# adaly/gridnext

Measured on AMD Instinct MI355X. Metric: spots/sec training throughput (multimodal f+g), higher is better.
Workload: dtype f32; 1 GPU; C4: multimodal f(DenseNet-121 @128px + count-MLP 2000 genes) + hex g on 78x64 Visium grids, 1 array (4992 spots) per GPU per step, f frozen/eval (tutorial mode), g trained with Adam, masked CE; spots_per_array=4992, parallelism=dp1

## Files before the change

### gridnext_amd/_lib.py

```python
import ctypes
import os

import torch

_HERE = os.path.dirname(os.path.abspath(__file__))
LIB_PATH = os.environ.get('GNX_LIB') or os.path.join(_HERE, 'libgridnext_hip.so')

_P, _I, _L, _F, _D = ctypes.c_void_p, ctypes.c_int, ctypes.c_long, ctypes.c_float, ctypes.c_double

SIGNATURES = {
    'gnx_hexconv_fwd': (_I, [_P, _P, _P, _P, _P, _I, _I, _I, _I, _I, _I, _P]),
    'gnx_hexconv_bwd_data': (_I, [_P, _P, _P, _P, _I, _I, _I, _I, _I, _I, _P]),
    'gnx_hexconv_bwd_weight_workspace': (_L, [_I, _I, _I, _I, _I]),
    'gnx_hexconv_bwd_weight': (_I, [_P, _P, _P, _P, _P, _P, _I, _I, _I, _I, _I, _I, _I, _P]),
    'gnx_hexconv_bwd_weight_batch': (_I, [_P, _I, _P]),
    'gnx_hexconv_k_fwd': (_I, [_P, _P, _P, _P, _I, _I, _I, _I, _I, _I, _I, _P]),
    'gnx_hexconv_k_bwd_data': (_I, [_P, _P, _P, _I, _I, _I, _I, _I, _I, _I, _P]),
    'gnx_hexconv_k_bwd_weight_workspace': (_L, [_I, _I, _I, _I, _I, _I]),
    'gnx_hexconv_k_bwd_weight': (_I, [_P, _P, _P, _P, _P, _I, _I, _I, _I, _I, _I, _I, _I, _P]),
    'gnx_bn_workspace': (_L, [_L, _I]),
    'gnx_bn_train_stats': (_I, [_P, _L, _L, _I, _P, _P, _P, _P, _P, _F, _F, _P, _P, _P, _P, _P, _P]),
    'gnx_bn_train_stats_sync': (_I, [_P, _L, _L, _I, _P, _P, _P, _P, _P, _F, _F, _P, _P, _P, _P, _P, _P, _P]),
    'gnx_bn_train_stats_apply': (_I, [_P, _L, _L, _I, _P, _P, _P, _P, _P, _F, _F, _P, _P, _P, _P, _P, _L, _I, _P, _P]),
    'gnx_bn_sync_words': (_L, [_I]),
# ... 78 lines not shown
    'gnx_conv_stem_bnrelu_maxpool_f16mul_cb': (_I, [_P, _I, _P, _P, _L, _L, _I, _I, _I, _I, _I, _I, _I, _I, _P, _P, _P, _P]),
    'gnx_conv1x1_bnrelu_h16_cb': (_I, [_P, _L, _P, _P, _L, _L, _I, _I, _P, _P, _P, _P, _P]),
    'gnx_bnrelu_avgpool2_h16_cb': (_I, [_P, _L, _P, _L, _L, _I, _I, _P, _P, _P]),
    'gnx_transition_f16_pack': (_I, [_P, _P, _I, _I, _P]),
    'gnx_transition_f16': (_I, [_P, _L, _L, _I, _I, _I, _P, _P, _P, _P, _L, _P]),
    'gnx_transition_f16_tape': (_I, [_P, _L, _L, _I, _I, _I, _P, _P, _P, _P, _L, _P, _L, _P]),
    'gnx_bnrelu_avgpool_h16_cb': (_I, [_P, _L, _P, _L, _L, _I, _I, _P, _P, _P]),
    'gnx_conv3x3_bnrelu': (_I, [_P, _L, _P, _P, _L, _L, _I, _I, _I, _P, _P, _P]),
    'gnx_winograd_conv3x3_weights': (_I, [_P, _P, _I, _I, _P]),
    'gnx_conv3x3_winograd': (_I, [_P, _L, _P, _P, _L, _L, _I, _I, _I, _P]),
    'gnx_conv_stem': (_I, [_P, _P, _P, _L, _L, _I, _I, _I, _I, _I, _I, _I, _I, _P]),
    'gnx_conv_stem_bnrelu_maxpool': (_I, [_P, _P, _P, _L, _L, _I, _I, _I, _I, _I, _I, _I, _I, _P, _P, _P]),
    'gnx_conv_stem_bnrelu_maxpool_argmax': (_I, [_P, _P, _P, _L, _P, _L, _I, _I, _I, _I, _I, _I, _I, _I, _P, _P, _P]),
    'gnx_bnrelu_maxpool': (_I, [_P, _L, _P, _L, _L, _I, _I, _I, _P, _P, _P]),
    'gnx_bnrelu_avgpool': (_I, [_P, _L, _P, _L, _L, _I, _I, _P, _P, _P]),
    'gnx_wgrad_workspace': (_L, [_L, _I, _I, _I]),
    'gnx_wgrad_bnrelu': (_I, [_P, _L, _P, _L, _P, _P, _P, _P, _L, _I, _I, _I, _I, _I, _I, _P]),
    'gnx_wgrad_bnrelu_batch': (_I, [_P, _I, _I, _P]),
    'gnx_transpose_weight': (_I, [_P, _P, _I, _I, _P]),
    'gnx_relayout_weights_batch': (_I, [_P, _I, _I, _P]),
    'gnx_repack_conv3x3_bwd': (_I, [_P, _P, _I, _I, _P]),
    'gnx_rows_broadcast': (_I, [_P, _L, _P, _L, _L, _I, _I, _F, _P]),
    'gnx_avgpool2_bwd': (_I, [_P, _L, _P, _L, _L, _I, _I, _P]),
    'gnx_maxpool_bwd': (_I, [_P, _L, _P, _L, _P, _L, _P, _L, _L, _I, _I, _I, _P, _P, _P]),
    'gnx_bnrelu_maxpool_argmax': (_I, [_P, _L, _P, _L, _P, _L, _I, _I, _I, _P, _P, _P]),
    'gnx_maxpool_bwd_argmax': (_I, [_P, _P, _L, _P, _L, _L, _I, _I, _I, _P]),
    'gnx_maxpool_bwd_argmax_bnrelu': (_I, [_P, _P, _L, _P, _L, _P, _P, _L, _L, _I, _I, _I, _P]),
    'gnx_conv0_wgrad_workspace': (_L, [_L, _I, _I, _I, _I, _I, _I, _I]),
    'gnx_conv0_wgrad': (_I, [_P, _P, _L, _P, _P, _L, _I, _I, _I, _I, _I, _I, _I, _I, _P]),
    'gnx_softmax_rows': (_I, [_P, _L, _L, _I, _P, _L, _P, _P]),
# ... 62 lines not shown
```

### gridnext_amd/csrc/stem_pool.hip

```cpp
#include <type_traits>
#include "fwd_common.h"

namespace {

__device__ __forceinline__ float u8_unit(float u) {
    constexpr float R255 = 1.0f / 255.0f;
    const float q = u * R255;
    const float e = fmaf(-255.0f, q, u);
    return fmaf(e, R255, q);
}
__device__ __forceinline__ float u8_pixel(float u, bool norm, float mean, float sd, float rsd) {
    float v = u8_unit(u);
    if (norm) {
        const float t = v - mean;
        const float q = t * rsd;
        const float e = fmaf(-sd, q, t);
        v = fmaf(e, rsd, q);
    }
    return v;
}
__device__ __forceinline__ float4 u8x4_pixels(uint32_t wv, bool norm, float mean, float sd, float rsd) {
    return make_float4(u8_pixel((float)(wv & 0xffu), norm, mean, sd, rsd),
                       u8_pixel((float)((wv >> 8) & 0xffu), norm, mean, sd, rsd),
                       u8_pixel((float)((wv >> 16) & 0xffu), norm, mean, sd, rsd),
// ... 178 lines not shown
                if (i < O) o[i] = acc0[r];
                if (32 + i < O) o[32 + i] = acc1[r];
            }
        }
    }
}

constexpr int SP_LDT = 40;
constexpr int SP_LDTH = 72;
template <int WO, bool H16 = false, bool U8 = false, bool IDX = false>
__global__ __launch_bounds__(256) void conv_stem_pool_kernel(const void* __restrict__ xv, const float* __restrict__ w,
                                                             float* __restrict__ out, long ldo, int H, int Wd, int O,
                                                             const float* __restrict__ scale,
                                                             const float* __restrict__ shift, long imgs,
                                                             const float* __restrict__ nrm,
                                                             unsigned char* __restrict__ amax = nullptr) {
    const float* __restrict__ x = reinterpret_cast<const float*>(xv);
    const uint8_t* __restrict__ x8 = reinterpret_cast<const uint8_t*>(xv);
    constexpr int CIN = 3, KH = 7, KW = 7, STRIDE = 2, PAD = 3;
    constexpr int RT = 128 / WO;
    constexpr int PH = STRIDE * (RT - 1) + KH, PW = ((WO - 1) * STRIDE + 8 + 1 + 1) & ~1;
    constexpr int F4R = WO * STRIDE / 4;
    constexpr int NPC = CIN * PH * F4R, NPRE = (NPC + 255) / 256;
    constexpr int NIT = (WO / 2) * 8 / 256;
    constexpr int KT = CIN * KH * 8, LDB = KT + 4;
    extern __shared__ __attribute__((aligned(16))) float lds[];
    auto store4 = [](float* o, long off, const float4& v) {
        if constexpr (H16) {
            typedef _Float16 half4 __attribute__((ext_vector_type(4)));
            const half4 hv = {(_Float16)v.x, (_Float16)v.y, (_Float16)v.z, (_Float16)v.w};
            *reinterpret_cast<half4*>(reinterpret_cast<_Float16*>(o) + off) = hv;
// ... 51 lines not shown
            if (j < NPC) {
                float* d = Ps + (j / F4R) * PW + PAD + 4 * (j % F4R);
                if constexpr (U8) {
                    const int c = (j / F4R) / PH;
                    const bool norm = nrm != nullptr;
                    const float4 v = in8[q] ? u8x4_pixels(pre8[q], norm, norm ? nrm[c] : 0.f, norm ? nrm[3 + c] : 1.f,
                                                          norm ? nrm[6 + c] : 1.f)
                                            : make_float4(0.f, 0.f, 0.f, 0.f);
                    d[0] = v.x; d[1] = v.y; d[2] = v.z; d[3] = v.w;
                } else {
                    d[0] = pre[q].x; d[1] = pre[q].y; d[2] = pre[q].z; d[3] = pre[q].w;
                }
            }
        }
    };
    __syncthreads();
    fetch_patch(blockIdx.x, 0);

    for (long img = blockIdx.x; img < imgs; img += gridDim.x) {
        float4 carry[2][NIT], carry2[2][NIT];
        unsigned cidx[2][NIT], cidx2[2][NIT];
        const float c0v = IDX ? -1.f : 0.f;
#pragma unroll
        for (int q = 0; q < NIT; ++q) {
            carry[0][q] = carry[1][q] = carry2[0][q] = carry2[1][q] = make_float4(c0v, c0v, c0v, c0v);
            cidx[0][q] = cidx[1][q] = cidx2[0][q] = cidx2[1][q] = 0u;
        }
        for (int tt = 0; tt < ntt; ++tt) {
            __syncthreads();
            stash_patch();
            {
                long nimg = img;
                int nt2 = tt + 1;
                if (nt2 == ntt) { nt2 = 0; nimg += gridDim.x; }
                if (nimg >= imgs) nimg = blockIdx.x;
                fetch_patch(nimg, nt2);
            }
            asm volatile("" ::: "memory");
            __syncthreads();
            f32x16 acc0, acc1;
#pragma unroll
            for (int r = 0; r < 16; ++r) { acc0[r] = 0.f; acc1[r] = 0.f; }
            auto load_a = [&](int step) {
                const float* ap = pa + ((step / KH) * PH + (step % KH)) * PW;
                const float2 lo = *reinterpret_cast<const float2*>(ap);
                const float2 hi = *reinterpret_cast<const float2*>(ap + 2);
                return make_float4(lo.x, lo.y, hi.x, hi.y);
            };
            constexpr int NSTEP = CIN * KH;
            float4 a = load_a(0), b0 = ld4(pb), b1 = ld4(pb + 32 * LDB);
#pragma unroll
// ... 356 lines not shown
                    if (a2 > m.z) { m.z = a2; am = (am & 0xff00ffffu) | (li << 16); }
                    if (a3 > m.w) { m.w = a3; am = (am & 0x00ffffffu) | (li << 24); }
                } else {
                    m.x = fmaxf(m.x, a0); m.y = fmaxf(m.y, a1); m.z = fmaxf(m.z, a2); m.w = fmaxf(m.w, a3);
                }
            }
        }
        *reinterpret_cast<float4*>(out + row * ldo + c) = m;
        if (IDX) *reinterpret_cast<unsigned*>(amax + row * (4L * C4) + c) = am;
    }
}

template <bool IN16 = false>
__global__ __launch_bounds__(256) void bnrelu_avgpool_kernel(const float* __restrict__ in, long ldi, float* __restrict__ out,
                                                             long ldo, int C, int S2, const float* __restrict__ scale,
                                                             const float* __restrict__ shift, long ibs = 32) {
    __shared__ float red[4][64];
    const int cl = threadIdx.x & 63, rl = threadIdx.x >> 6;
    const int c = blockIdx.y * 64 + cl;
    const long img = blockIdx.x;
    float acc = 0.f;
    if (c < C) {
        const float sc = scale[c], sh = shift[c];
        for (int r = rl; r < S2; r += 4) {
            const long off = (img * S2 + r) * ldi + (c >> 5) * ibs + (c & 31);
            const float v = IN16 ? (float)reinterpret_cast<const _Float16*>(in)[off] : in[off];
            acc += fmaxf(fmaf(v, sc, sh), 0.f);
        }
    }
    red[rl][cl] = acc;
    __syncthreads();
    if (rl == 0 && c < C)
        out[img * ldo + c] = ((red[0][cl] + red[1][cl]) + (red[2][cl] + red[3][cl])) / (float)S2;
}

}

GNX_EXPORT int gnx_conv_stem(const float* x, const float* w, float* out, long ldc, long imgs, int Cin, int H, int W,
                             int O, int KH, int KW, int stride, int pad, hipStream_t stream) {
    if (!x || !w || !out || imgs < 0 || Cin <= 0 || O <= 0 || KH <= 0 || KH > 7 || KW <= 0 || KW > 8 || stride <= 0 ||
        ldc < O)
        return GNX_ERR_BAD_ARG;
    const int Ho = (H + 2 * pad - KH) / stride + 1, Wo = (W + 2 * pad - KW) / stride + 1;
    if (Ho <= 0 || Wo <= 0) return GNX_ERR_BAD_ARG;
    const long M = imgs * Ho * Wo;
    if (M == 0) return GNX_OK;
    if (O <= 64 && Cin == 3 && ((stride == 2 && KH == 7 && KW == 7) || (stride == 1 && KH == 3 && KW == 3))) {
        const int tiles_x = gnx_cdiv(Wo, 16), tiles_y = gnx_cdiv(Ho, 8);
// ... 6 lines not shown
                                                                      tiles_x, tiles_y, ntiles);
        else
            conv_stem_patch_kernel<1, 3, 3><<<grid2, 256, lds2, stream>>>(x, w, out, ldc, Cin, H, W, Ho, Wo, O, KW, pad,
                                                                      tiles_x, tiles_y, ntiles);
        return gnx_launch_status();
    }
    const size_t lds_bytes = (size_t)(ST_BM + ST_BN) * (KH * 8 + 4) * sizeof(float);
    dim3 grid(gnx_cdiv(M, ST_BM), gnx_cdiv(O, ST_BN));
    conv_stem_kernel<<<grid, 256, lds_bytes, stream>>>(x, w, out, ldc, M, Cin, H, W, Ho, Wo, O, KH, KW, stride, pad);
    return gnx_launch_status();
}

template <bool H16, bool U8 = false>
static int stem_pool_launch(const void* x, const float* w, float* out, long ldo, long imgs, int Cin, int H, int W, int O,
                            int KH, int KW, int stride, int pad, const float* scale, const float* shift, hipStream_t stream,
                            const float* nrm = nullptr, unsigned char* amax = nullptr) {
    if (!x || !w || !out || !scale || !shift || imgs < 0 || Cin <= 0 || O <= 0 || H <= 0 || W <= 0 || ldo < O)
        return GNX_ERR_BAD_ARG;
    if (amax && (H16 || U8 || (reinterpret_cast<uintptr_t>(amax) & 3) != 0)) return GNX_ERR_UNSUPPORTED;
    if (Cin != 3 || KH != 7 || KW != 7 || stride != 2 || pad != 3 || O > 64 || O % 4 != 0 || ldo % 4 != 0 ||
        (reinterpret_cast<uintptr_t>(out) & (H16 ? 7 : 15)) != 0)
        return GNX_ERR_UNSUPPORTED;
    const int Ho = (H + 6 - 7) / 2 + 1, Wo = (W + 6 - 7) / 2 + 1;
    if ((Wo != 64 && Wo != 128) || W != 2 * Wo || Ho % 2 != 0 || Ho <= 0 ||
        (reinterpret_cast<uintptr_t>(x) & (U8 ? 3 : 15)) != 0)
        return GNX_ERR_UNSUPPORTED;
    if (imgs == 0) return GNX_OK;
    const int RT = 128 / Wo, PH = 2 * (RT - 1) + 7, PW = ((Wo - 1) * 2 + 8 + 2) & ~1;
    const size_t lds_bytes = ((size_t)64 * (3 * 7 * 8 + 4) + (size_t)3 * PH * PW + (size_t)128 * SP_LDT) * sizeof(float);
    const int per_cu = lds_bytes <= 80 * 1024 ? 2 : 1;
    const int grid = (int)(imgs < 256 * per_cu ? imgs : 256 * per_cu);
    if (Wo == 64) {
        static bool conf = false;
// ... 5 lines not shown
        }
        if constexpr (!H16 && !U8) {
            if (amax) {
                static bool confi = false;
                if (!confi) {
                    if (hipFuncSetAttribute(reinterpret_cast<const void*>(conv_stem_pool_kernel<64, false, false, true>),
                                            hipFuncAttributeMaxDynamicSharedMemorySize, (int)lds_bytes) != hipSuccess)
                        return GNX_ERR_LAUNCH;
                    confi = true;
                }
                conv_stem_pool_kernel<64, false, false, true><<<grid, 256, lds_bytes, stream>>>(x, w, out, ldo, H, W, O, scale,
                                                                                                shift, imgs, nrm, amax);
                return gnx_launch_status();
            }
        }
        conv_stem_pool_kernel<64, H16, U8><<<grid, 256, lds_bytes, stream>>>(x, w, out, ldo, H, W, O, scale, shift, imgs, nrm);
    } else {
        static bool conf = false;
        if (!conf) {
            if (hipFuncSetAttribute(reinterpret_cast<const void*>(conv_stem_pool_kernel<128, H16, U8>),
                                    hipFuncAttributeMaxDynamicSharedMemorySize, (int)lds_bytes) != hipSuccess)
                return GNX_ERR_LAUNCH;
            conf = true;
        }
        if constexpr (!H16 && !U8) {
            if (amax) {
                static bool confi = false;
                if (!confi) {
                    if (hipFuncSetAttribute(reinterpret_cast<const void*>(conv_stem_pool_kernel<128, false, false, true>),
                                            hipFuncAttributeMaxDynamicSharedMemorySize, (int)lds_bytes) != hipSuccess)
                        return GNX_ERR_LAUNCH;
                    confi = true;
                }
                conv_stem_pool_kernel<128, false, false, true><<<grid, 256, lds_bytes, stream>>>(x, w, out, ldo, H, W, O, scale,
                                                                                                 shift, imgs, nrm, amax);
                return gnx_launch_status();
            }
        }
        conv_stem_pool_kernel<128, H16, U8><<<grid, 256, lds_bytes, stream>>>(x, w, out, ldo, H, W, O, scale, shift, imgs, nrm);
    }
    return gnx_launch_status();
}
GNX_EXPORT int gnx_conv_stem_bnrelu_maxpool(const float* x, const float* w, float* out, long ldo, long imgs, int Cin,
                                            int H, int W, int O, int KH, int KW, int stride, int pad, const float* scale,
                                            const float* shift, hipStream_t stream) {
    return stem_pool_launch<false>(x, w, out, ldo, imgs, Cin, H, W, O, KH, KW, stride, pad, scale, shift, stream);
}
GNX_EXPORT int gnx_conv_stem_bnrelu_maxpool_argmax(const float* x, const float* w, float* out, long ldo,
                                                   unsigned char* argmax, long imgs, int Cin, int H, int W, int O, int KH,
                                                   int KW, int stride, int pad, const float* scale, const float* shift,
                                                   hipStream_t stream) {
    if (!argmax) return GNX_ERR_BAD_ARG;
    return stem_pool_launch<false>(x, w, out, ldo, imgs, Cin, H, W, O, KH, KW, stride, pad, scale, shift, stream, nullptr,
                                   argmax);
}
GNX_EXPORT int gnx_conv_stem_bnrelu_maxpool_h16(const float* x, const float* w, void* out16, long ldo, long imgs, int Cin,
                                                int H, int W, int O, int KH, int KW, int stride, int pad,
                                                const float* scale, const float* shift, hipStream_t stream) {
    return stem_pool_launch<true>(x, w, reinterpret_cast<float*>(out16), ldo, imgs, Cin, H, W, O, KH, KW, stride, pad, scale,
                                  shift, stream);
}
// ... 44 lines not shown
    if (norm) return GNX_ERR_BAD_ARG;
    return stem_pool_f16_launch<false>(x, w, out16, 32, imgs, Cin, H, W, O, KH, KW, stride, pad, scale, shift, nullptr, stream,
                                       rows_total * 32);
}

GNX_EXPORT int gnx_conv_stem_bnrelu_maxpool_u8(const uint8_t* x8, const float* w, void* out, long ldo, long imgs, int Cin,
                                               int H, int W, int O, int KH, int KW, int stride, int pad, const float* scale,
                                               const float* shift, const float* norm, int out_f16, hipStream_t stream) {
    if (out_f16)
        return stem_pool_launch<true, true>(x8, w, reinterpret_cast<float*>(out), ldo, imgs, Cin, H, W, O, KH, KW, stride, pad,
                                            scale, shift, stream, norm);
    return stem_pool_launch<false, true>(x8, w, reinterpret_cast<float*>(out), ldo, imgs, Cin, H, W, O, KH, KW, stride, pad,
                                         scale, shift, stream, norm);
}

GNX_EXPORT int gnx_u8_to_f32(const uint8_t* x8, float* out, long imgs, int C, int H, int W, const float* norm,
                             hipStream_t stream) {
    if (!x8 || !out || imgs < 0 || C <= 0 || H <= 0 || W <= 0 || (norm && C != 3)) return GNX_ERR_BAD_ARG;
    const long hw = (long)H * W;
    if (hw % 4 != 0 || (reinterpret_cast<uintptr_t>(x8) & 3) != 0 || !al16(out)) return GNX_ERR_UNSUPPORTED;
    const long n4 = imgs * C * hw / 4;
    if (n4 == 0) return GNX_OK;
    const long blocks = (n4 + 255) / 256;
    u8_to_f32_kernel<<<(int)(blocks < 256 * 16 ? blocks : 256 * 16), 256, 0, stream>>>(x8, out, n4, hw / 4, C, norm);
    return gnx_launch_status();
}

static int bnrelu_maxpool_launch(const float* in, long ldi, float* out, long ldo, unsigned char* amax, long imgs, int C,
                                 int Hi, int Wi, const float* scale, const float* shift, hipStream_t stream) {
    if (!in || !out || !scale || !shift || imgs < 0 || C <= 0 || Hi <= 0 || Wi <= 0 || ldi < C || ldo < C)
// ... 29 lines not shown
GNX_EXPORT int gnx_bnrelu_maxpool_argmax(const float* in, long ldi, float* out, long ldo, unsigned char* argmax, long imgs,
                                         int C, int Hi, int Wi, const float* scale, const float* shift, hipStream_t stream) {
    if (!argmax) return GNX_ERR_BAD_ARG;
    return bnrelu_maxpool_launch(in, ldi, out, ldo, argmax, imgs, C, Hi, Wi, scale, shift, stream);
}

GNX_EXPORT int gnx_bnrelu_avgpool(const float* in, long ldi, float* out, long ldo, long imgs, int C, int S2,
                                  const float* scale, const float* shift, hipStream_t stream) {
    if (!in || !out || !scale || !shift || imgs < 0 || C <= 0 || S2 <= 0 || ldi < C || ldo < C) return GNX_ERR_BAD_ARG;
    if (imgs == 0) return GNX_OK;
    if (imgs > 2147483647L) return GNX_ERR_UNSUPPORTED;
    dim3 grid((unsigned)imgs, gnx_cdiv(C, 64));
    bnrelu_avgpool_kernel<false><<<grid, 256, 0, stream>>>(in, ldi, out, ldo, C, S2, scale, shift);
    return gnx_launch_status();
}
GNX_EXPORT int gnx_bnrelu_avgpool_h16(const void* in16, long ldi, float* out, long ldo, long imgs, int C, int S2,
                                      const float* scale, const float* shift, hipStream_t stream) {
    if (!in16 || !out || !scale || !shift || imgs < 0 || C <= 0 || S2 <= 0 || ldi < C || ldo < C) return GNX_ERR_BAD_ARG;
    if (imgs == 0) return GNX_OK;
    if (imgs > 2147483647L) return GNX_ERR_UNSUPPORTED;
    dim3 grid((unsigned)imgs, gnx_cdiv(C, 64));
    bnrelu_avgpool_kernel<true><<<grid, 256, 0, stream>>>(reinterpret_cast<const float*>(in16), ldi, out, ldo, C, S2, scale,
                                                          shift);
    return gnx_launch_status();
}
GNX_EXPORT int gnx_bnrelu_avgpool_h16_cb(const void* in16, long rows_total, float* out, long ldo, long imgs, int C, int S2,
                                         const float* scale, const float* shift, hipStream_t stream) {
    if (!in16 || !out || !scale || !shift || imgs < 0 || C <= 0 || S2 <= 0 || rows_total < imgs * S2 || ldo < C || C % 32 != 0)
        return GNX_ERR_BAD_ARG;
    if (imgs == 0) return GNX_OK;
// ... 7 lines not shown
```

### gridnext_amd/densenet.py

```python
import math
from collections import OrderedDict
from types import SimpleNamespace

import torch
import torch.nn as nn

from . import _lib as L
from . import functional as GF

F32 = torch.float32


class _DenseLayer(nn.Module):
    def __init__(self, c_in, growth_rate, bn_size, drop_rate):
        super().__init__()
        self.norm1 = nn.BatchNorm2d(c_in)
        self.relu1 = nn.ReLU(inplace=True)
        self.conv1 = nn.Conv2d(c_in, bn_size * growth_rate, kernel_size=1, stride=1, bias=False)
        self.norm2 = nn.BatchNorm2d(bn_size * growth_rate)
        self.relu2 = nn.ReLU(inplace=True)
        self.conv2 = nn.Conv2d(bn_size * growth_rate, growth_rate, kernel_size=3, stride=1, padding=1, bias=False)
        self.drop_rate = drop_rate


class _Transition(nn.Module):
# ... 10 lines not shown
                 num_init_features=24, bn_size=4, drop_rate=0,
                 num_classes=10, small_inputs=True, efficient=False, classify=True):
        super().__init__()
        assert 0 < compression <= 1, 'compression of densenet should be between 0 and 1'
        self.drop_rate = float(drop_rate or 0)
        self.growth_rate, self.block_config = growth_rate, tuple(block_config)
        self.bn_size, self.small_inputs, self.classify = bn_size, small_inputs, classify
        self.efficient = bool(efficient)
        self.tape_budget = 150 * 1024 ** 3
        self.atonce = None
        self.mfma = 'f32'
        self.split_conv1 = False
        self.split_conv2 = False
        self.split_wgrad = False
        self.winograd = True
        self.f16_buffers = True
        self.f16_stem = True
        self.f16_fused = True
        self.f16_fused_transitions = True
        self.f16_fused_conv2_backward = True
        self.input_norm = None

        feats = OrderedDict()
        if small_inputs:
            feats['conv0'] = nn.Conv2d(3, num_init_features, kernel_size=3, stride=1, padding=1, bias=False)
        else:
            feats['conv0'] = nn.Conv2d(3, num_init_features, kernel_size=7, stride=2, padding=3, bias=False)
            feats['norm0'] = nn.BatchNorm2d(num_init_features)
            feats['relu0'] = nn.ReLU(inplace=True)
            feats['pool0'] = nn.MaxPool2d(kernel_size=3, stride=2, padding=1, ceil_mode=False)
# ... 222 lines not shown
    def _probe_begin(self):
        if self._probe is None:
            return None
        ev = torch.cuda.Event(enable_timing=True)
        ev.record()
        return ev

    def _probe_mark(self, kind, start, flops=None, nbytes=None):
        if self._probe is None:
            return None
        ev = torch.cuda.Event(enable_timing=True)
        ev.record()
        self._probe.append((kind, start, ev, flops, nbytes))
        return ev

    def _stem_eval(self, xu, rows, c_total, P, hs, use_h, fold, w0, stem_out, chunk, st):
        nu = xu.shape[0]
        dev = xu.device
        c0 = self.features.conv0.out_channels
        if self.small_inputs:
            xu = self._float_patches(xu)
            L.call('gnx_conv_stem', L.ptr(xu), L.ptr(w0), L.ptr(rows), c_total, nu, 3, P, P, c0, 3, 3, 1, 1, st)
            return stem_out
        sc, sh = fold[self.features.norm0]
        u8 = xu.dtype == torch.uint8
        if use_h and self.f16_stem and L.try_call(
                'gnx_conv_stem_bnrelu_maxpool_f16mul', xu.data_ptr(), 1 if u8 else 0, L.ptr(w0), rows.data_ptr(), c_total, nu, 3,
                P, P, c0, 7, 7, 2, 3, L.ptr(sc), L.ptr(sh), L.ptr(self._norm_vector(dev)) if u8 else None, st):
            return stem_out
        if u8:
            if L.try_call('gnx_conv_stem_bnrelu_maxpool_u8', xu.data_ptr(), L.ptr(w0), rows.data_ptr(), c_total, nu, 3, P, P,
                          c0, 7, 7, 2, 3, L.ptr(sc), L.ptr(sh), L.ptr(self._norm_vector(dev)), 1 if use_h else 0, st):
                return stem_out
            xu = self._float_patches(xu)
# ... 77 lines not shown
            self.growth_rate == 32 and mid % 128 == 0 and N % 8 == 0 and maps_ok
        chunk = self._auto_chunk(P, N, 2 if h_shapes else 4)

        def whole_groups(g):
            lim = min((2 ** 31 - 1) // (s * s * max(mid, c_total)) for (_, _, _, c_total), s in zip(self._blocks, sizes))
            return max(g, min(chunk, lim) // g * g)
        if not f16 and self.atonce is None and 128 <= chunk < N:
            chunk = whole_groups(128)
        if f16 and self.atonce is None and chunk >= 8:
            chunk = chunk // 8 * 8 if (fused_ok and h_shapes) else whole_groups(8)
        use_h = h_shapes and chunk % 8 == 0 and \
            (fused_ok or all(min(chunk, N) * s * s * max(mid, c_total) < 2 ** 31
                             for (_, _, _, c_total), s in zip(self._blocks, sizes)))
        return chunk, use_h, use_h and fused_ok

    @torch.no_grad()
    def _forward_eval(self, x):
        x = x.contiguous() if x.dtype == torch.uint8 else x.contiguous().float()
        N, _, P, _ = x.shape
        chunk, use_h, fused = self._eval_plan(N, P)
        self._used_f16_buffers, self._used_f16_fused = use_h, fused
        f32, mid = self.mfma == 'f32', self.bn_size * self.growth_rate
        w = SimpleNamespace(
            fold=self._folded_eval(), w2=self._repacked_conv2(),
            w2u=self._winograd_conv2() if (self.winograd and f32) else None,
            w2h=self._repacked_conv2_f16() if not f32 else None,
            w1s=self._split_conv1() if (self.split_conv1 and f32 and mid == 128) else None,
            w2s=self._split_conv2() if (self.split_conv2 and f32 and mid == 128 and self.growth_rate == 32) else None,
            w1h=self._conv1_f16() if (use_h and not fused) else None,
            dlp=self._dense_f16_packed() if fused else None)
        dev = x.device
        hs, sizes = self._geometry(P)
        if fused:
            bufs = [torch.empty((c_total // 32, chunk * s * s, 32), device=dev, dtype=torch.float16)
                    for (_, _, _, c_total), s in zip(self._blocks, sizes)]
        else:
            bufs = [torch.empty((chunk * s * s, c_total), device=dev, dtype=torch.float16 if use_h else F32)
                    for (_, _, _, c_total), s in zip(self._blocks, sizes)]
        bott = torch.empty((1 if fused else chunk * sizes[0] * sizes[0], mid), device=dev, dtype=F32)
        stem_out = None
        feats = torch.empty((N, self.num_features), device=dev, dtype=F32)
        w0 = self.features.conv0.weight.detach().contiguous()
        st = L.stream()
        for s0 in range(0, N, chunk):
            n = min(chunk, N - s0)
            xs = x[s0:s0 + n]
            for bi, ((c_in, layers, trans, c_total), s) in enumerate(zip(self._blocks, sizes)):
                nxt = bufs[bi + 1] if trans is not None else None
                if fused:
                    self._block_fused(bi, bufs[bi], nxt, xs, n, s, P, w.fold, w0, w.dlp, st)
                    continue
                rows = bufs[bi][:n * s * s]
                if bi == 0:
                    stem_out = self._stem_eval(xs, rows, c_total, P, hs, use_h, w.fold, w0, stem_out, chunk, st)
                for li, layer in enumerate(layers):
                    self._layer_eval(layer, rows, c_total, c_in + li * self.growth_rate, n, s, use_h, w, bott, st)
                if trans is not None:
                    self._transition_eval(trans, rows, nxt, c_total, n, s, use_h, w.fold, st)
            self._tail_eval(bufs[-1], feats[s0:], n, sizes[-1], use_h, fused, w.fold, st)
        if not self.classify:
            return feats
        return GF.linear(feats, self.classifier.weight.detach(), self.classifier.bias.detach())

    def _layer_eval(self, layer, rows, c_total, cin, n, s, use_h, w, bott, st):
        M, mid, g = n * s * s, self.bn_size * self.growth_rate, self.growth_rate
        bn1, bn2 = w.fold[layer.norm1], w.fold[layer.norm2]
        if self.mfma == 'f32':
            dense_layer_f32_act(self, layer, rows, c_total, cin, bott, M, s, bn1, bn2, w.w2[layer], w.w1s, w.w2s, w.w2u, st)
            return
        H = torch.float16
        bott16 = bott.view(H)
        dma = use_h or self._f16_dma_ok(M, s, mid, c_total)
        eb, em = (2 if use_h else 4), (2 if dma else 4)
        t0 = self._probe_begin()
# ... 67 lines not shown
```

### include/gridnext_hip.h

```cpp
#ifndef GRIDNEXT_HIP_H
#define GRIDNEXT_HIP_H

#ifdef __cplusplus
extern "C" {
#endif

#define GNX_OK 0
#define GNX_ERR_BAD_ARG (-1)
#define GNX_ERR_LAUNCH (-2)
#define GNX_ERR_UNSUPPORTED (-3)

typedef void* gnx_stream_t;

int gnx_hexconv_fwd(const float* x, const float* kernel0, const float* kernel1, const float* bias, float* y,
                    int B, int H, int W, int I, int O, int mode, gnx_stream_t stream);
int gnx_hexconv_bwd_data(const float* dy, const float* kernel0, const float* kernel1, float* dx,
                         int B, int H, int W, int I, int O, int mode, gnx_stream_t stream);
long gnx_hexconv_bwd_weight_workspace(int B, int H, int W, int I, int O);
int gnx_hexconv_bwd_weight(const float* x, const float* dy, float* dkernel0, float* dkernel1, float* dbias,
                           float* workspace, int B, int H, int W, int I, int O, int mode, int accumulate,
                           gnx_stream_t stream);
typedef struct {
    const float* x; const float* dy; float* dkernel0; float* dkernel1; float* dbias; float* workspace;
    int B, H, W, I, O, mode, accumulate, pad;
// ... 114 lines not shown
int gnx_winograd_conv3x3_weights(const float* w, float* wu, int N, int K, gnx_stream_t stream);
int gnx_conv3x3_winograd(const float* A, long lda, const float* Wu, float* out, long ldc, long M, int N, int K, int S,
                         gnx_stream_t stream);
int gnx_conv_stem(const float* x, const float* w, float* out, long ldc, long imgs, int Cin, int H, int W, int O,
                  int KH, int KW, int stride, int pad, gnx_stream_t stream);
int gnx_conv_stem_bnrelu_maxpool(const float* x, const float* w, float* out, long ldo, long imgs, int Cin, int H, int W,
                                 int O, int KH, int KW, int stride, int pad, const float* scale, const float* shift,
                                 gnx_stream_t stream);
int gnx_conv_stem_bnrelu_maxpool_argmax(const float* x, const float* w, float* out, long ldo, unsigned char* argmax,
                                        long imgs, int Cin, int H, int W, int O, int KH, int KW, int stride, int pad,
                                        const float* scale, const float* shift, gnx_stream_t stream);
int gnx_bnrelu_maxpool(const float* in, long ldi, float* out, long ldo, long imgs, int C, int Hi, int Wi,
                       const float* scale, const float* shift, gnx_stream_t stream);
int gnx_bnrelu_avgpool(const float* in, long ldi, float* out, long ldo, long imgs, int C, int S2,
                       const float* scale, const float* shift, gnx_stream_t stream);

int gnx_conv1x1_bnrelu_f16(const float* A, long lda, const float* W, float* out, long ldc, long M, int N, int K,
                           const float* scale, const float* shift, int pool, int S_in, gnx_stream_t stream);
int gnx_conv3x3_bnrelu_f16(const float* A, long lda, const float* Wr, float* out, long ldc, long M, int N, int K, int S,
                           const float* scale, const float* shift, gnx_stream_t stream);
int gnx_conv1x1_bnrelu_f16_act16(const float* A, long lda, const float* W, void* out16, long ldc16, long M, int N, int K,
                                 const float* scale, const float* shift, const float* out_scale, const float* out_shift,
                                 gnx_stream_t stream);
int gnx_conv3x3_f16_dma(const void* A16, long lda16, const void* Wr16, float* out, long ldc, long M, int N, int K, int S,
                        gnx_stream_t stream);
int gnx_conv_stem_bnrelu_maxpool_h16(const float* x, const float* w, void* out16, long ldo, long imgs, int Cin, int H, int W,
                                     int O, int KH, int KW, int stride, int pad, const float* scale, const float* shift,
                                     gnx_stream_t stream);
int gnx_conv_stem_bnrelu_maxpool_u8(const unsigned char* x8, const float* w, void* out, long ldo, long imgs, int Cin, int H,
                                    int W, int O, int KH, int KW, int stride, int pad, const float* scale,
// ... 133 lines not shown
```

Before: 79150 spots/s.

## Skip all-zero spots in frozen DenseNet eval and broadcast one shared feature

Adds a scan kernel that flags all-zero spot images and a single-block compaction kernel that builds foreground and background index lists. The frozen DenseNet forward then runs only on the foreground spots plus one representative empty spot. The stem reads through a gather index, the final BN-ReLU-avgpool scatters results to the original rows, and one broadcast kernel copies the empty-spot feature to every other empty row. This removes redundant CNN work on padded or empty grid positions. In exchange it adds a host sync (.item()) for the count, is gated on f32 MFMA and specific shapes, and its interaction with the fused path looks unclear.

Result: faster. 84760 spots/s (median of 6 runs) (+7.1%).

```diff
diff --git a/gridnext_amd/_lib.py b/gridnext_amd/_lib.py
--- a/gridnext_amd/_lib.py
+++ b/gridnext_amd/_lib.py
@@ -116,6 +116,11 @@
     'gnx_conv_stem_bnrelu_maxpool_argmax': (_I, [_P, _P, _P, _L, _P, _L, _I, _I, _I, _I, _I, _I, _I, _I, _P, _P, _P]),
     'gnx_bnrelu_maxpool': (_I, [_P, _L, _P, _L, _L, _I, _I, _I, _P, _P, _P]),
     'gnx_bnrelu_avgpool': (_I, [_P, _L, _P, _L, _L, _I, _I, _P, _P, _P]),
+    'gnx_spot_compact': (_I, [_P, _L, _L, _P, _P, _P, _P, _P]),
+    'gnx_spot_broadcast_rows': (_I, [_P, _L, _L, _I, _P, _L, _P]),
+    'gnx_conv_stem_bnrelu_maxpool_idx': (_I, [_P, _P, _P, _L, _L, _I, _I, _I, _I, _I, _I, _I, _I, _P, _P, _P, _L, _P]),
+    'gnx_conv_stem_bnrelu_maxpool_u8_idx': (_I, [_P, _P, _P, _L, _L, _I, _I, _I, _I, _I, _I, _I, _I, _P, _P, _P, _P, _L, _P]),
+    'gnx_bnrelu_avgpool_idx': (_I, [_P, _L, _P, _L, _L, _I, _I, _P, _P, _P, _L, _P]),
     'gnx_wgrad_workspace': (_L, [_L, _I, _I, _I]),
     'gnx_wgrad_bnrelu': (_I, [_P, _L, _P, _L, _P, _P, _P, _P, _L, _I, _I, _I, _I, _I, _I, _P]),
     'gnx_wgrad_bnrelu_batch': (_I, [_P, _I, _I, _P]),
diff --git a/gridnext_amd/csrc/spot_compact.hip b/gridnext_amd/csrc/spot_compact.hip
--- /dev/null
+++ b/gridnext_amd/csrc/spot_compact.hip
@@ -0,0 +1,95 @@
+#include "common.h"
+
+namespace {
+
+constexpr int SC_UNR = 4;
+
+__global__ __launch_bounds__(256) void spot_scan_kernel(const uint4* __restrict__ x, long q16, int* __restrict__ empty) {
+    const uint4* __restrict__ p = x + (long)blockIdx.x * q16;
+    const int t = threadIdx.x;
+    int nonzero = 0;
+    long base = 0;
+    for (int unr = 1; base < q16 && !nonzero; base += 256L * unr, unr = SC_UNR) {
+        unsigned acc = 0u;
+#pragma unroll
+        for (int u = 0; u < SC_UNR; ++u) {
+            const long j = base + 256L * u + t;
+            if (u < unr && j < q16) {
+                const uint4 v = p[j];
+                acc |= v.x | v.y | v.z | v.w;
+            }
+        }
+        nonzero = __syncthreads_or(acc != 0u);
+    }
+    if (t == 0) empty[blockIdx.x] = nonzero ? 0 : 1;
+}
+
+__global__ __launch_bounds__(1024) void spot_compact_kernel(const int* __restrict__ empty, long N, int* __restrict__ fg_idx,
+                                                            int* __restrict__ bg_idx, int* __restrict__ counts) {
+    __shared__ int wf[16], wb[16], first_bg;
+    const int t = threadIdx.x, lane = t & 63, wid = t >> 6;
+    if (t == 0) first_bg = 0;
+    long nf = 0, nb = 0;
+    for (long start = 0; start < N; start += 1024) {
+        const long i = start + t;
+        const int e = i < N ? empty[i] : -1;
+        const unsigned long long mf = __ballot(e == 0), mb = __ballot(e == 1);
+        const unsigned long long below = (1ull << lane) - 1ull;
+        __syncthreads();
+        if (lane == 0) { wf[wid] = __popcll(mf); wb[wid] = __popcll(mb); }
+        __syncthreads();
+        int of = 0, ob = 0, tf = 0, tb = 0;
+#pragma unroll
+        for (int k = 0; k < 16; ++k) {
+            if (k < wid) { of += wf[k]; ob += wb[k]; }
+            tf += wf[k]; tb += wb[k];
+        }
+        if (e == 0) fg_idx[nf + of + __popcll(mf & below)] = (int)i;
+        if (e == 1) {
+            const long pos = nb + ob + __popcll(mb & below);
+            bg_idx[pos] = (int)i;
+            if (pos == 0) first_bg = (int)i;
+        }
+        nf += tf;
+        nb += tb;
+    }
+    __syncthreads();
+    const int fill = first_bg;
+    for (long j = nf + t; j < N; j += 1024) fg_idx[j] = fill;
+    if (t == 0) { counts[0] = (int)nf; counts[1] = (int)nb; }
+}
+
+__global__ __launch_bounds__(256) void spot_broadcast_rows_kernel(float* __restrict__ rows, long ld, int C,
+                                                                  const int* __restrict__ bg_idx, long n_bg, long n_rows) {
+    const long src = bg_idx[0];
+    if (src < 0 || src >= n_rows) return;
+    const long total = (n_bg - 1) * C;
+    for (long k = (long)blockIdx.x * blockDim.x + threadIdx.x; k < total; k += (long)gridDim.x * blockDim.x) {
+        const long r = k / C;
+        const int c = (int)(k - r * C);
+        const long dst = bg_idx[1 + r];
+        if (dst >= 0 && dst < n_rows) rows[dst * ld + c] = rows[src * ld + c];
+    }
+}
+
+}
+
+GNX_EXPORT int gnx_spot_compact(const void* x, long spot_bytes, long N, int* flags, int* fg_idx, int* bg_idx, int* counts,
+                                hipStream_t stream) {
+    if (!x || !flags || !fg_idx || !bg_idx || !counts || spot_bytes <= 0 || N < 0) return GNX_ERR_BAD_ARG;
+    if (spot_bytes % 16 != 0 || (reinterpret_cast<uintptr_t>(x) & 15) != 0 || N > 2147483647L) return GNX_ERR_UNSUPPORTED;
+    if (N > 0)
+        spot_scan_kernel<<<(unsigned)N, 256, 0, stream>>>(reinterpret_cast<const uint4*>(x), spot_bytes / 16, flags);
+    spot_compact_kernel<<<1, 1024, 0, stream>>>(flags, N, fg_idx, bg_idx, counts);
+    return gnx_launch_status();
+}
+
+GNX_EXPORT int gnx_spot_broadcast_rows(float* rows, long ld, long n_rows, int C, const int* bg_idx, long n_bg,
+                                       hipStream_t stream) {
+    if (!rows || !bg_idx || ld < C || C <= 0 || n_rows <= 0 || n_bg < 0 || n_bg > n_rows) return GNX_ERR_BAD_ARG;
+    if (n_bg <= 1) return GNX_OK;
+    long blocks = ((n_bg - 1) * C + 255) / 256;
+    if (blocks > 4096) blocks = 4096;
+    spot_broadcast_rows_kernel<<<(unsigned)blocks, 256, 0, stream>>>(rows, ld, C, bg_idx, n_bg, n_rows);
+    return gnx_launch_status();
+}
diff --git a/gridnext_amd/csrc/stem_pool.hip b/gridnext_amd/csrc/stem_pool.hip
--- a/gridnext_amd/csrc/stem_pool.hip
+++ b/gridnext_amd/csrc/stem_pool.hip
@@ -216,7 +216,8 @@
                                                              const float* __restrict__ scale,
                                                              const float* __restrict__ shift, long imgs,
                                                              const float* __restrict__ nrm,
-                                                             unsigned char* __restrict__ amax = nullptr) {
+                                                             unsigned char* __restrict__ amax = nullptr,
+                                                             const int* __restrict__ src_idx = nullptr, long src_imgs = 0) {
     const float* __restrict__ x = reinterpret_cast<const float*>(xv);
     const uint8_t* __restrict__ x8 = reinterpret_cast<const uint8_t*>(xv);
     constexpr int CIN = 3, KH = 7, KW = 7, STRIDE = 2, PAD = 3;
@@ -298,10 +299,16 @@
             }
         }
     };
+    auto src_of = [&](long img) -> long {
+        if (src_idx == nullptr) return img;
+        const long s = src_idx[img];
+        return s < 0 ? 0 : (s < src_imgs ? s : src_imgs - 1);
+    };
     __syncthreads();
-    fetch_patch(blockIdx.x, 0);
+    fetch_patch(src_of(blockIdx.x), 0);
 
     for (long img = blockIdx.x; img < imgs; img += gridDim.x) {
+        const long src = src_of(img);
         float4 carry[2][NIT], carry2[2][NIT];
         unsigned cidx[2][NIT], cidx2[2][NIT];
         const float c0v = IDX ? -1.f : 0.f;
@@ -314,11 +321,15 @@
             __syncthreads();
             stash_patch();
             {
-                long nimg = img;
+                long nsrc = src;
                 int nt2 = tt + 1;
-                if (nt2 == ntt) { nt2 = 0; nimg += gridDim.x; }
-                if (nimg >= imgs) nimg = blockIdx.x;
-                fetch_patch(nimg, nt2);
+                if (nt2 == ntt) {
+                    nt2 = 0;
+                    long nimg = img + gridDim.x;
+                    if (nimg >= imgs) nimg = blockIdx.x;
+                    nsrc = src_of(nimg);
+                }
+                fetch_patch(nsrc, nt2);
             }
             asm volatile("" ::: "memory");
             __syncthreads();
@@ -705,7 +716,8 @@
 template <bool IN16 = false>
 __global__ __launch_bounds__(256) void bnrelu_avgpool_kernel(const float* __restrict__ in, long ldi, float* __restrict__ out,
                                                              long ldo, int C, int S2, const float* __restrict__ scale,
-                                                             const float* __restrict__ shift, long ibs = 32) {
+                                                             const float* __restrict__ shift, long ibs = 32,
+                                                             const int* __restrict__ dst_idx = nullptr, long dst_rows = 0) {
     __shared__ float red[4][64];
     const int cl = threadIdx.x & 63, rl = threadIdx.x >> 6;
     const int c = blockIdx.y * 64 + cl;
@@ -721,8 +733,14 @@
     }
     red[rl][cl] = acc;
     __syncthreads();
-    if (rl == 0 && c < C)
-        out[img * ldo + c] = ((red[0][cl] + red[1][cl]) + (red[2][cl] + red[3][cl])) / (float)S2;
+    if (rl == 0 && c < C) {
+        long orow = img;
+        if (dst_idx != nullptr) {
+            orow = dst_idx[img];
+            if (orow < 0 || orow >= dst_rows) return;
+        }
+        out[orow * ldo + c] = ((red[0][cl] + red[1][cl]) + (red[2][cl] + red[3][cl])) / (float)S2;
+    }
 }
 
 }
@@ -759,9 +777,11 @@
 template <bool H16, bool U8 = false>
 static int stem_pool_launch(const void* x, const float* w, float* out, long ldo, long imgs, int Cin, int H, int W, int O,
                             int KH, int KW, int stride, int pad, const float* scale, const float* shift, hipStream_t stream,
-                            const float* nrm = nullptr, unsigned char* amax = nullptr) {
+                            const float* nrm = nullptr, unsigned char* amax = nullptr, const int* src_idx = nullptr,
+                            long src_imgs = 0) {
     if (!x || !w || !out || !scale || !shift || imgs < 0 || Cin <= 0 || O <= 0 || H <= 0 || W <= 0 || ldo < O)
         return GNX_ERR_BAD_ARG;
+    if (src_idx && (src_imgs <= 0 || amax)) return GNX_ERR_BAD_ARG;
     if (amax && (H16 || U8 || (reinterpret_cast<uintptr_t>(amax) & 3) != 0)) return GNX_ERR_UNSUPPORTED;
     if (Cin != 3 || KH != 7 || KW != 7 || stride != 2 || pad != 3 || O > 64 || O % 4 != 0 || ldo % 4 != 0 ||
         (reinterpret_cast<uintptr_t>(out) & (H16 ? 7 : 15)) != 0)
@@ -797,7 +817,8 @@
                 return gnx_launch_status();
             }
         }
-        conv_stem_pool_kernel<64, H16, U8><<<grid, 256, lds_bytes, stream>>>(x, w, out, ldo, H, W, O, scale, shift, imgs, nrm);
+        conv_stem_pool_kernel<64, H16, U8><<<grid, 256, lds_bytes, stream>>>(x, w, out, ldo, H, W, O, scale, shift, imgs, nrm,
+                                                                             nullptr, src_idx, src_imgs);
     } else {
         static bool conf = false;
         if (!conf) {
@@ -820,7 +841,8 @@
                 return gnx_launch_status();
             }
         }
-        conv_stem_pool_kernel<128, H16, U8><<<grid, 256, lds_bytes, stream>>>(x, w, out, ldo, H, W, O, scale, shift, imgs, nrm);
+        conv_stem_pool_kernel<128, H16, U8><<<grid, 256, lds_bytes, stream>>>(x, w, out, ldo, H, W, O, scale, shift, imgs, nrm,
+                                                                              nullptr, src_idx, src_imgs);
     }
     return gnx_launch_status();
 }
@@ -828,6 +850,13 @@
                                             int H, int W, int O, int KH, int KW, int stride, int pad, const float* scale,
                                             const float* shift, hipStream_t stream) {
     return stem_pool_launch<false>(x, w, out, ldo, imgs, Cin, H, W, O, KH, KW, stride, pad, scale, shift, stream);
+}
+GNX_EXPORT int gnx_conv_stem_bnrelu_maxpool_idx(const float* x, const float* w, float* out, long ldo, long imgs, int Cin,
+                                                int H, int W, int O, int KH, int KW, int stride, int pad, const float* scale,
+                                                const float* shift, const int* src_idx, long src_imgs, hipStream_t stream) {
+    if (!src_idx) return GNX_ERR_BAD_ARG;
+    return stem_pool_launch<false>(x, w, out, ldo, imgs, Cin, H, W, O, KH, KW, stride, pad, scale, shift, stream, nullptr,
+                                   nullptr, src_idx, src_imgs);
 }
 GNX_EXPORT int gnx_conv_stem_bnrelu_maxpool_argmax(const float* x, const float* w, float* out, long ldo,
                                                    unsigned char* argmax, long imgs, int Cin, int H, int W, int O, int KH,
@@ -902,6 +931,15 @@
                                          scale, shift, stream, norm);
 }
 
+GNX_EXPORT int gnx_conv_stem_bnrelu_maxpool_u8_idx(const uint8_t* x8, const float* w, float* out, long ldo, long imgs, int Cin,
+                                                   int H, int W, int O, int KH, int KW, int stride, int pad, const float* scale,
+                                                   const float* shift, const float* norm, const int* src_idx, long src_imgs,
+                                                   hipStream_t stream) {
+    if (!src_idx) return GNX_ERR_BAD_ARG;
+    return stem_pool_launch<false, true>(x8, w, out, ldo, imgs, Cin, H, W, O, KH, KW, stride, pad, scale, shift, stream, norm,
+                                         nullptr, src_idx, src_imgs);
+}
+
 GNX_EXPORT int gnx_u8_to_f32(const uint8_t* x8, float* out, long imgs, int C, int H, int W, const float* norm,
                              hipStream_t stream) {
     if (!x8 || !out || imgs < 0 || C <= 0 || H <= 0 || W <= 0 || (norm && C != 3)) return GNX_ERR_BAD_ARG;
@@ -961,6 +999,17 @@
     bnrelu_avgpool_kernel<false><<<grid, 256, 0, stream>>>(in, ldi, out, ldo, C, S2, scale, shift);
     return gnx_launch_status();
 }
+GNX_EXPORT int gnx_bnrelu_avgpool_idx(const float* in, long ldi, float* out, long ldo, long imgs, int C, int S2,
+                                      const float* scale, const float* shift, const int* dst_idx, long dst_rows,
+                                      hipStream_t stream) {
+    if (!in || !out || !scale || !shift || !dst_idx || dst_rows <= 0 || imgs < 0 || C <= 0 || S2 <= 0 || ldi < C || ldo < C)
+        return GNX_ERR_BAD_ARG;
+    if (imgs == 0) return GNX_OK;
+    if (imgs > 2147483647L) return GNX_ERR_UNSUPPORTED;
+    dim3 grid((unsigned)imgs, gnx_cdiv(C, 64));
+    bnrelu_avgpool_kernel<false><<<grid, 256, 0, stream>>>(in, ldi, out, ldo, C, S2, scale, shift, 32, dst_idx, dst_rows);
+    return gnx_launch_status();
+}
 GNX_EXPORT int gnx_bnrelu_avgpool_h16(const void* in16, long ldi, float* out, long ldo, long imgs, int C, int S2,
                                       const float* scale, const float* shift, hipStream_t stream) {
     if (!in16 || !out || !scale || !shift || imgs < 0 || C <= 0 || S2 <= 0 || ldi < C || ldo < C) return GNX_ERR_BAD_ARG;
diff --git a/gridnext_amd/densenet.py b/gridnext_amd/densenet.py
--- a/gridnext_amd/densenet.py
+++ b/gridnext_amd/densenet.py
@@ -9,6 +9,31 @@
 from . import functional as GF
 
 F32 = torch.float32
+
+EMPTY_GRANULE = 8
+
+
+def compacted_spots(N, n_fg, chunk, granule=EMPTY_GRANULE):
+    if n_fg >= N:
+        return None
+    n_c = n_fg + 1
+    n_c += (N - n_c) % granule
+    if n_c >= N:
+        return None
+    if not (chunk >= N or (chunk % granule == 0 and N % granule == 0)):
+        return None
+    return n_c
+
+
+def empty_spot_lists(x):
+    N = x.shape[0]
+    ws = torch.empty(3 * N + 2, device=x.device, dtype=torch.int32)
+    flags, fg, bg, counts = ws[:N], ws[N:2 * N], ws[2 * N:3 * N], ws[3 * N:]
+    I32 = torch.int32
+    if not L.try_call('gnx_spot_compact', x.data_ptr(), x[0].numel() * x.element_size() if N else 16, N, L.ptr(flags, I32),
+                      L.ptr(fg, I32), L.ptr(bg, I32), L.ptr(counts, I32), L.stream()):
+        return None
+    return fg, bg, counts
 
 
 class _DenseLayer(nn.Module):
@@ -49,6 +74,7 @@
         self.split_conv2 = False
         self.split_wgrad = False
         self.winograd = True
+        self.skip_empty = True
         self.f16_buffers = True
         self.f16_stem = True
         self.f16_fused = True
@@ -301,10 +327,19 @@
         self._probe.append((kind, start, ev, flops, nbytes))
         return ev
 
-    def _stem_eval(self, xu, rows, c_total, P, hs, use_h, fold, w0, stem_out, chunk, st):
+    def _stem_eval(self, xu, rows, c_total, P, hs, use_h, fold, w0, stem_out, chunk, st, src=None, n_src=0):
         nu = xu.shape[0]
         dev = xu.device
         c0 = self.features.conv0.out_channels
+        if src is not None:
+            sc, sh = fold[self.features.norm0]
+            if xu.dtype == torch.uint8:
+                L.call('gnx_conv_stem_bnrelu_maxpool_u8_idx', xu.data_ptr(), L.ptr(w0), L.ptr(rows), c_total, n_src, 3, P, P, c0,
+                       7, 7, 2, 3, L.ptr(sc), L.ptr(sh), L.ptr(self._norm_vector(dev)), L.ptr(src, torch.int32), nu, st)
+            else:
+                L.call('gnx_conv_stem_bnrelu_maxpool_idx', L.ptr(xu), L.ptr(w0), L.ptr(rows), c_total, n_src, 3, P, P, c0, 7, 7,
+                       2, 3, L.ptr(sc), L.ptr(sh), L.ptr(src, torch.int32), nu, st)
+            return stem_out
         if self.small_inputs:
             xu = self._float_patches(xu)
             L.call('gnx_conv_stem', L.ptr(xu), L.ptr(w0), L.ptr(rows), c_total, nu, 3, P, P, c0, 3, 3, 1, 1, st)
@@ -412,11 +447,36 @@
                              for (_, _, _, c_total), s in zip(self._blocks, sizes)))
         return chunk, use_h, use_h and fused_ok
 
+    def _skip_empty_shapes(self, x, P):
+        c0 = self.features.conv0.out_channels
+        hs, sizes = self._geometry(P)
+        return (self.mfma == 'f32' and not self.small_inputs and P in (128, 256) and c0 <= 64 and c0 % 4 == 0 and
+                self.features.conv0.kernel_size == (7, 7) and all(s in (4, 8, 16, 32, 64) for s in sizes) and
+                all(c_total % 4 == 0 for _, _, _, c_total in self._blocks) and
+                x.data_ptr() % (4 if x.dtype == torch.uint8 else 16) == 0)
+
+    def _compact_empty(self, x, N, P, chunk):
+        if not self.skip_empty or N <= EMPTY_GRANULE or not self._skip_empty_shapes(x, P) or \
+                torch.cuda.is_current_stream_capturing():
+            return None
+        lists = empty_spot_lists(x)
+        if lists is None:
+            return None
+        fg, bg, counts = lists
+        n_fg = int(counts[0].item())
+        n = compacted_spots(N, n_fg, chunk)
+        return None if n is None else SimpleNamespace(fg=fg, bg=bg, n_fg=n_fg, n=n)
+
     @torch.no_grad()
     def _forward_eval(self, x):
         x = x.contiguous() if x.dtype == torch.uint8 else x.contiguous().float()
         N, _, P, _ = x.shape
         chunk, use_h, fused = self._eval_plan(N, P)
+        empty = self._compact_empty(x, N, P, chunk)
+        Nc = N if empty is None else empty.n
+        if empty is not None:
+            chunk = self._eval_plan(Nc, P)[0]
+        self._skipped_empty = 0 if empty is None else N - Nc
         self._used_f16_buffers, self._used_f16_fused = use_h, fused
         f32, mid = self.mfma == 'f32', self.bn_size * self.growth_rate
         w = SimpleNamespace(
@@ -440,9 +500,10 @@
         feats = torch.empty((N, self.num_features), device=dev, dtype=F32)
         w0 = self.features.conv0.weight.detach().contiguous()
         st = L.stream()
-        for s0 in range(0, N, chunk):
-            n = min(chunk, N - s0)
-            xs = x[s0:s0 + n]
+        for s0 in range(0, Nc, chunk):
+            n = min(chunk, Nc - s0)
+            xs = x[s0:s0 + n] if empty is None else x
+            src = None if empty is None else empty.fg[s0:s0 + n]
             for bi, ((c_in, layers, trans, c_total), s) in enumerate(zip(self._blocks, sizes)):
                 nxt = bufs[bi + 1] if trans is not None else None
                 if fused:
@@ -450,12 +511,21 @@
                     continue
                 rows = bufs[bi][:n * s * s]
                 if bi == 0:
-                    stem_out = self._stem_eval(xs, rows, c_total, P, hs, use_h, w.fold, w0, stem_out, chunk, st)
+                    stem_out = self._stem_eval(xs, rows, c_total, P, hs, use_h, w.fold, w0, stem_out, chunk, st, src, n)
                 for li, layer in enumerate(layers):
                     self._layer_eval(layer, rows, c_total, c_in + li * self.growth_rate, n, s, use_h, w, bott, st)
                 if trans is not None:
                     self._transition_eval(trans, rows, nxt, c_total, n, s, use_h, w.fold, st)
-            self._tail_eval(bufs[-1], feats[s0:], n, sizes[-1], use_h, fused, w.fold, st)
+            if empty is None:
+                self._tail_eval(bufs[-1], feats[s0:], n, sizes[-1], use_h, fused, w.fold, st)
+            elif s0 <= empty.n_fg:
+                scf, shf = w.fold[self.features.norm_final]
+                L.call('gnx_bnrelu_avgpool_idx', L.ptr(bufs[-1]), bufs[-1].shape[1], L.ptr(feats), self.num_features,
+                       min(n, empty.n_fg + 1 - s0), self.num_features, sizes[-1] ** 2, L.ptr(scf), L.ptr(shf),
+                       L.ptr(src, torch.int32), N, st)
+        if empty is not None:
+            L.call('gnx_spot_broadcast_rows', L.ptr(feats), self.num_features, N, self.num_features,
+                   L.ptr(empty.bg, torch.int32), N - empty.n_fg, st)
         if not self.classify:
             return feats
         return GF.linear(feats, self.classifier.weight.detach(), self.classifier.bias.detach())
diff --git a/include/gridnext_hip.h b/include/gridnext_hip.h
--- a/include/gridnext_hip.h
+++ b/include/gridnext_hip.h
@@ -152,6 +152,19 @@
                        const float* scale, const float* shift, gnx_stream_t stream);
 int gnx_bnrelu_avgpool(const float* in, long ldi, float* out, long ldo, long imgs, int C, int S2,
                        const float* scale, const float* shift, gnx_stream_t stream);
+
+int gnx_spot_compact(const void* x, long spot_bytes, long N, int* flags, int* fg_idx, int* bg_idx, int* counts,
+                     gnx_stream_t stream);
+int gnx_spot_broadcast_rows(float* rows, long ld, long n_rows, int C, const int* bg_idx, long n_bg, gnx_stream_t stream);
+int gnx_conv_stem_bnrelu_maxpool_idx(const float* x, const float* w, float* out, long ldo, long imgs, int Cin, int H, int W,
+                                     int O, int KH, int KW, int stride, int pad, const float* scale, const float* shift,
+                                     const int* src_idx, long src_imgs, gnx_stream_t stream);
+int gnx_conv_stem_bnrelu_maxpool_u8_idx(const unsigned char* x8, const float* w, float* out, long ldo, long imgs, int Cin,
+                                        int H, int W, int O, int KH, int KW, int stride, int pad, const float* scale,
+                                        const float* shift, const float* norm, const int* src_idx, long src_imgs,
+                                        gnx_stream_t stream);
+int gnx_bnrelu_avgpool_idx(const float* in, long ldi, float* out, long ldo, long imgs, int C, int S2, const float* scale,
+                           const float* shift, const int* dst_idx, long dst_rows, gnx_stream_t stream);
 
 int gnx_conv1x1_bnrelu_f16(const float* A, long lda, const float* W, float* out, long ldc, long M, int N, int K,
                            const float* scale, const float* shift, int pool, int S_in, gnx_stream_t stream);
```
